# SauersML/genomic_pca

Measured on AMD Instinct MI355X. Metric: SNPs x samples / sec through rSVD at k=20; max|dPC| vs ref, higher is better.
Workload: dtype i8 (exact: int8 dosages x 4 signed 7-bit fixed-point digit planes of the skinny operand, i32 accumulate, f64 recombination; accuracy >= f32)

## Files before the change

### genomic_pca_amd/csrc/kernels.hip

```cpp
#include "kernels.h"
#include "philox.hpp"
#include "omega_math.h"

#ifndef GPCA_OMEGA_ABLATE
#define GPCA_OMEGA_ABLATE 0
#endif
namespace gpca {

__device__ const OmegaLnEntry kOmegaLnTable[kOmegaLnEntries] = {
#include "omega_table.inc"
};

typedef float f32x16 __attribute__((ext_vector_type(16)));

#define DEVINL __device__ __forceinline__

__global__ __launch_bounds__(256) void k_synth(int8_t* __restrict__ G, int64_t M, int64_t N, int64_t ld,
                                                int64_t snp_offset, uint64_t seed,
                                                const uint32_t* __restrict__ thresh, int P) {
    const int64_t per_row = ld >> 3;
    const int64_t t = (int64_t)blockIdx.x * 256 + threadIdx.x;
    if (t >= M * per_row) return;
    const int64_t i = t / per_row;
    const int64_t n0 = (t - i * per_row) << 3;
// ... 548 lines not shown
    const int64_t r0 = (int64_t)blockIdx.x * rpb;
    const int64_t r1 = (r0 + rpb < rows) ? r0 + rpb : rows;
    TX xc[4][G], xn[4][G];
    auto load_rows = [&](int64_t n, TX (&dst)[4][G]) {
#pragma unroll
        for (int u = 0; u < 4; ++u) {
            const int64_t row = n + 4 * u + k;
#pragma unroll
            for (int g = 0; g < G; ++g) dst[u][g] = row < r1 ? X[row * L + 16 * g + i] : (TX)0;
        }
    };
    load_rows(r0 + 16 * wv, xc);
    for (int64_t n = r0 + 16 * wv; n < r1; n += 64) {
        load_rows(n + 64, xn);
#pragma unroll
        for (int u = 0; u < 4; ++u) {
            double x[G];
#pragma unroll
            for (int g = 0; g < G; ++g) x[g] = (double)xc[u][g];
            int t = 0;
#pragma unroll
            for (int ga = 0; ga < G; ++ga)
#pragma unroll
                for (int gc = ga; gc < G; ++gc, ++t)
                    acc[t] = __builtin_amdgcn_mfma_f64_16x16x4f64(x[ga], x[gc], acc[t], 0, 0, 0);
        }
#pragma unroll
        for (int u = 0; u < 4; ++u)
#pragma unroll
            for (int g = 0; g < G; ++g) xc[u][g] = xn[u][g];
    }
    if (wv > 0) {
#pragma unroll
        for (int t = 0; t < NT; ++t)
#pragma unroll
            for (int r = 0; r < 4; ++r) red[wv - 1][t][lane][r] = acc[t][r];
    }
    __syncthreads();
    if (wv != 0) return;
    double* out = part + (int64_t)blockIdx.x * L * L;
    int t = 0;
#pragma unroll
    for (int ga = 0; ga < G; ++ga)
#pragma unroll
        for (int gc = ga; gc < G; ++gc, ++t)
#pragma unroll
            for (int r = 0; r < 4; ++r) {
                const double v = ((acc[t][r] + red[0][t][lane][r]) + red[1][t][lane][r]) + red[2][t][lane][r];
                const int a = 16 * ga + 4 * r + k, c = 16 * gc + i;
                out[a * L + c] = v;
                if (ga != gc) out[c * L + a] = v;
            }
}
void launch_gram_f64(hipStream_t st, const double* X, int64_t rows, int L, double* part) {
    const int64_t rpb = gram_rows_per_block(rows);
    const dim3 grid((unsigned)gram_num_parts(rows)), blk(256);
    if (L == 32) hipLaunchKernelGGL((k_gram_mfma<double, 32>), grid, blk, 0, st, X, rows, rpb, part);
    else if (L == 64) hipLaunchKernelGGL((k_gram_mfma<double, 64>), grid, blk, 0, st, X, rows, rpb, part);
    else launch_gram_any_f64(st, X, rows, rpb, gram_num_parts(rows), L, part);
}
void launch_gram_f32(hipStream_t st, const float* X, int64_t rows, int L, double* part) {
    const int64_t rpb = gram_rows_per_block(rows);
    const dim3 grid((unsigned)gram_num_parts(rows)), blk(256);
    if (L == 32) hipLaunchKernelGGL((k_gram_mfma<float, 32>), grid, blk, 0, st, X, rows, rpb, part);
    else if (L == 64) hipLaunchKernelGGL((k_gram_mfma<float, 64>), grid, blk, 0, st, X, rows, rpb, part);
    else launch_gram_any_f32(st, X, rows, rpb, gram_num_parts(rows), L, part);
}

template <int L>
__global__ __launch_bounds__(256) void k_apply_right(double* __restrict__ X, int64_t rows, const double* __restrict__ Z,
                                                     float* __restrict__ Qout, int64_t rows_pad) {
    constexpr int RPB = 256 / L;
    __shared__ double zs[L][L + 1];
    __shared__ double xs[RPB][L];
    for (int e = threadIdx.x; e < L * L; e += 256) zs[e / L][e % L] = Z[e];
    const int rr = threadIdx.x / L, cc = threadIdx.x % L;
    const int64_t n = (int64_t)blockIdx.x * RPB + rr;
    xs[rr][cc] = (n < rows) ? X[n * L + cc] : 0.0;
    __syncthreads();
    double a = 0.0;
#pragma unroll 8
    for (int j = 0; j < L; ++j) a += xs[rr][j] * zs[j][cc];
    if (n < rows) X[n * L + cc] = a;
    if (Qout && n < rows_pad) Qout[blocked_q_index(n, cc, L >> 5)] = (n < rows) ? (float)a : 0.f;
}
constexpr int kTailRows = 64;
int64_t tail_num_parts(int64_t rows_pad) { return (rows_pad + kTailRows - 1) / kTailRows; }
template <int L>
__global__ __launch_bounds__(256) void k_apply_right_tail(double* __restrict__ X, int64_t rows, const double* __restrict__ Z,
                                                          float* __restrict__ Qout, int64_t rows_pad,
                                                          double* __restrict__ csum_part, double* __restrict__ amax_part) {
    constexpr int RPB = 256 / L;
    __shared__ double zs[L][L + 1];
    __shared__ double xs[RPB][L];
    __shared__ double red[2][RPB][L];
    for (int e = threadIdx.x; e < L * L; e += 256) zs[e / L][e % L] = Z[e];
    const int rr = threadIdx.x / L, cc = threadIdx.x % L;
    double cs = 0.0, am = 0.0;
    const int64_t n0 = (int64_t)blockIdx.x * kTailRows;
    for (int sub = 0; sub < kTailRows; sub += RPB) {
        const int64_t n = n0 + sub + rr;
        __syncthreads();
        xs[rr][cc] = (n < rows) ? X[n * L + cc] : 0.0;
        __syncthreads();
        double a = 0.0;
#pragma unroll 8
        for (int j = 0; j < L; ++j) a += xs[rr][j] * zs[j][cc];
        if (n < rows) { X[n * L + cc] = a; cs += a; am = fmax(am, fabs(a)); }
        if (Qout && n < rows_pad) Qout[blocked_q_index(n, cc, L >> 5)] = (n < rows) ? (float)a : 0.f;
    }
    red[0][rr][cc] = cs; red[1][rr][cc] = am;
    __syncthreads();
    if (rr == 0) {
        for (int g = 1; g < RPB; ++g) { cs += red[0][g][cc]; am = fmax(am, red[1][g][cc]); }
        csum_part[(int64_t)blockIdx.x * L + cc] = cs;
        amax_part[(int64_t)blockIdx.x * L + cc] = am;
    }
}
void launch_apply_right_tail(hipStream_t st, double* X, int64_t rows, int L, const double* Z, float* Qout, int64_t rows_pad,
                             double* csum_part, double* amax_part) {
    const dim3 grid((unsigned)tail_num_parts(rows_pad)), blk(256);
    if (L == 32) hipLaunchKernelGGL((k_apply_right_tail<32>), grid, blk, 0, st, X, rows, Z, Qout, rows_pad, csum_part, amax_part);
    else if (L == 64) hipLaunchKernelGGL((k_apply_right_tail<64>), grid, blk, 0, st, X, rows, Z, Qout, rows_pad, csum_part, amax_part);
    else launch_apply_right_any(st, X, rows, tail_num_parts(rows_pad), L, Z, csum_part, amax_part);
}
__global__ __launch_bounds__(1024) void k_finish_q(const double* __restrict__ csum_part, const double* __restrict__ amax_part,
                                                   int64_t P, int L, double* __restrict__ s64, float* __restrict__ s32,
                                                   double* __restrict__ scale, double* __restrict__ inv, double S) {
    __shared__ double rs[1024], rm[1024];
    const int cc = threadIdx.x % L, pg = threadIdx.x / L, G = 1024 / L;
    double a = 0.0, m = 0.0;
    for (int64_t p = pg; p < P; p += G) { a += csum_part[p * L + cc]; m = fmax(m, amax_part[p * L + cc]); }
    rs[threadIdx.x] = a; rm[threadIdx.x] = m;
    __syncthreads();
    if (pg != 0) return;
    for (int g = 1; g < G; ++g) { a += rs[g * L + cc]; m = fmax(m, rm[g * L + cc]); }
    s64[cc] = a; s32[cc] = (float)a;
    if (scale) { scale[cc] = m > 0.0 ? m / S : 0.0; inv[cc] = m > 0.0 ? S / m : 0.0; }
}
void launch_finish_q(hipStream_t st, const double* csum_part, const double* amax_part, int64_t P, int L, double* s64, float* s32,
                     double* scale, double* inv, int nd) {
    hipLaunchKernelGGL(k_finish_q, dim3(1), dim3(1024), 0, st, csum_part, amax_part, P, L, s64, s32, scale, inv, digit_scale(nd));
}

constexpr double kCholRankTol = 1e-13;
__device__ __forceinline__ double rsqrt_nr(double x) {
    double y = __builtin_amdgcn_rsq(x);
    y = y * (1.5 - 0.5 * x * y * y);
    y = y * (1.5 - 0.5 * x * y * y);
    return y;
}
__device__ __forceinline__ double bcast_lane(double v, int lane) {
    return __hiloint2double(__builtin_amdgcn_readlane(__double2hiint(v), lane), __builtin_amdgcn_readlane(__double2loint(v), lane));
}
__device__ __forceinline__ void wave_lds_sync() { __builtin_amdgcn_fence(__ATOMIC_RELEASE, "wavefront"); __builtin_amdgcn_wave_barrier(); __builtin_amdgcn_fence(__ATOMIC_ACQUIRE, "wavefront"); }
template <int NN>
__device__ __forceinline__ void chol_inv_wave(const double* Wg, int n, double* __restrict__ Zg, int* __restrict__ flag, double* rs, int c) {
    double col[NN], x[NN], dinv[NN];
#pragma unroll
    for (int r = 0; r < NN; ++r) col[r] = Wg[r * NN + (c & (NN - 1))];
#pragma unroll
    for (int r = 0; r < NN; ++r) col[r] = (r < n && c < n) ? col[r] : ((r == c) ? 1.0 : 0.0);
    double diag0 = 0.0;
#pragma unroll
    for (int r = 0; r < NN; ++r) diag0 = (r == c) ? col[r] : diag0;
#pragma unroll
    for (int j = 0; j < NN; ++j) {
        __builtin_amdgcn_sched_barrier(0);
        double piv = bcast_lane(col[j], j);
        const double d0 = bcast_lane(diag0, j);
        if (!isfinite(piv) || !isfinite(d0)) {
            if (c == 0) atomicCAS(flag, 0, j + 1);
            piv = 1.0;
        }
        const bool dependent = !(piv > kCholRankTol * d0);
        dinv[j] = dependent ? 0.0 : rsqrt_nr(piv);
        col[j] = (c == j) ? piv * dinv[j] : col[j] * dinv[j];
        if (c < NN) rs[j * NN + c] = col[j];
        wave_lds_sync();
        double row[NN];
#pragma unroll
        for (int r = j + 1; r < NN; ++r) row[r] = rs[j * NN + r];
#pragma unroll
        for (int r = j + 1; r < NN; ++r) asm volatile("" : "+v"(row[r]));
#pragma unroll
        for (int r = j + 1; r < NN; ++r) { col[r] -= row[r] * col[j]; asm volatile("" : "+v"(col[r])); }
    }
#pragma unroll
    for (int i = NN - 1; i >= 0; --i) {
        __builtin_amdgcn_sched_barrier(0);
        double acc = (c == i) ? 1.0 : 0.0;
#pragma unroll
        for (int k = i + 1; k < NN; ++k) acc -= rs[i * NN + k] * x[k];
        x[i] = acc * dinv[i];
        asm volatile("" : "+v"(x[i]));
    }
    if (c < NN) {
#pragma unroll
        for (int i = 0; i < NN; ++i) Zg[i * NN + c] = (i < n && c < n) ? x[i] : 0.0;
    }
}
template <int NN>
__global__ __launch_bounds__(64) void k_chol_inv(const double* __restrict__ Wg, int n, double* __restrict__ Zg,
                                                 int* __restrict__ flag) {
    __shared__ double rs[NN * NN];
    chol_inv_wave<NN>(Wg, n, Zg, flag, rs, (int)threadIdx.x);
}
__global__ __launch_bounds__(256) void k_chol_inv_fold32(const double* __restrict__ part, int P, int n, double* __restrict__ Zg, int* __restrict__ flag) {
    __shared__ double rs[32 * 32];
    double a[4] = {0.0, 0.0, 0.0, 0.0};
    for (int p0 = 0; p0 < P; p0 += 16) {
        double v[4][16];
#pragma unroll
        for (int u = 0; u < 16; ++u) {
            const double* pp = part + (size_t)(p0 + u < P ? p0 + u : p0) * 1024 + threadIdx.x;
#pragma unroll
            for (int q = 0; q < 4; ++q) v[q][u] = pp[256 * q];
        }
#pragma unroll
        for (int u = 0; u < 16; ++u)
#pragma unroll
            for (int q = 0; q < 4; ++q) a[q] += (p0 + u < P) ? v[q][u] : 0.0;
    }
#pragma unroll
    for (int q = 0; q < 4; ++q) rs[threadIdx.x + 256 * q] = a[q];
    __syncthreads();
    if (threadIdx.x >= 64) return;
    chol_inv_wave<32>(rs, n, Zg, flag, rs, (int)threadIdx.x);
}
void launch_chol_inv_fold(hipStream_t st, const double* part, int P, int n, int ld, double* Z, int* flag) {
    (void)ld;
    hipLaunchKernelGGL(k_chol_inv_fold32, dim3(1), dim3(256), 0, st, part, P, n, Z, flag);
}
void launch_chol_inv(hipStream_t st, const double* W, int n, int ld, double* Z, int* flag) {
    if (ld == 32) hipLaunchKernelGGL(k_chol_inv<32>, dim3(1), dim3(64), 0, st, W, n, Z, flag);
    else if (ld == 64) hipLaunchKernelGGL(k_chol_inv<64>, dim3(1), dim3(64), 0, st, W, n, Z, flag);
    else (void)launch_chol_inv_any(st, W, n, ld, Z, flag);
}

void launch_apply_right_inplace(hipStream_t st, double* X, int64_t rows, int L, const double* Z, float* Qout,
                                int64_t rows_pad) {
    const int64_t span = Qout ? rows_pad : rows;
    if (L == 32) hipLaunchKernelGGL((k_apply_right<32>), dim3((unsigned)((span + 7) / 8)), dim3(256), 0, st, X, rows, Z, Qout, rows_pad);
    else if (L == 64) hipLaunchKernelGGL((k_apply_right<64>), dim3((unsigned)((span + 3) / 4)), dim3(256), 0, st, X, rows, Z, Qout, rows_pad);
    else launch_apply_right_any(st, X, rows, (rows + 63) / 64, L, Z, nullptr, nullptr);
}

template <typename TX, int L>
__global__ __launch_bounds__(256) void k_rightmul(const TX* __restrict__ X, const int64_t* __restrict__ row_ids,
                                                  int64_t nrows, const double* __restrict__ Z, int K,
                                                  double* __restrict__ out64, float* __restrict__ out32) {
    extern __shared__ double zsm[];
    float* osm = reinterpret_cast<float*>(zsm + L * K);
    const int KP = K | 1;
    for (int e = threadIdx.x; e < L * K; e += 256) zsm[e] = Z[e];
    __syncthreads();
    const int64_t n0 = (int64_t)blockIdx.x * 256;
    const int64_t n = n0 + threadIdx.x;
    if (n < nrows) {
        const int64_t src = row_ids ? row_ids[n] : n;
        double x[L];
#pragma unroll
        for (int j = 0; j < L; ++j) x[j] = (double)X[src * L + j];
        for (int kc = 0; kc < K; ++kc) {
            double a = 0.0;
#pragma unroll
            for (int j = 0; j < L; ++j) a += x[j] * zsm[j * K + kc];
            if (out64) out64[n * K + kc] = a;
            if (out32) osm[threadIdx.x * KP + kc] = (float)a;
        }
    }
    if (!out32) return;
    __syncthreads();
    const int64_t rows_here = (nrows - n0 < 256) ? nrows - n0 : 256;
    const int total = (int)rows_here * K;
    float* dst = out32 + n0 * K;
    for (int e = threadIdx.x; e < total; e += 256) dst[e] = osm[(e / K) * KP + (e % K)];
}
static size_t rightmul_lds(int L, int K, bool f32out) { return sizeof(double) * L * K + (f32out ? sizeof(float) * 256 * (size_t)(K | 1) : 0); }
void launch_rightmul_f64(hipStream_t st, const double* X, int64_t rows, int L, const double* Z, int K, double* out64,
                         float* out32) {
    const dim3 grid((unsigned)((rows + 255) / 256)), blk(256);
    const size_t lds = rightmul_lds(L, K, out32 != nullptr);
    if (L == 32) hipLaunchKernelGGL((k_rightmul<double, 32>), grid, blk, lds, st, X, (const int64_t*)nullptr, rows, Z, K, out64, out32);
    else if (L == 64) {
        hipLaunchKernelGGL((k_rightmul<double, 64>), grid, blk, lds, st, X, (const int64_t*)nullptr, rows, Z, K, out64, out32);
    } else launch_rightmul_any_f64(st, X, rows, L, Z, K, out64, out32);
}
template <int L, int NJ>
__global__ __launch_bounds__(256) void k_rightmul_mfma(const float* __restrict__ X, const int64_t* __restrict__ row_ids,
                                                       int64_t nrows, const double* __restrict__ Z, int K,
                                                       float* __restrict__ out32, int64_t tiles_per_wave, const int* __restrict__ sign) {
    constexpr int E = L / 4;
    const int lane = threadIdx.x & 63, wv = threadIdx.x >> 6;
    const int i = lane & 15, kq = lane >> 4;
    double zb[E][NJ];
#pragma unroll
    for (int jt = 0; jt < NJ; ++jt) {
        const int col = 16 * jt + i;
        const double sg = (sign && col < K) ? (double)sign[col] : 1.0;
#pragma unroll
        for (int s2 = 0; s2 < E; ++s2) zb[s2][jt] = col < K ? Z[(E * kq + s2) * K + col] * sg : 0.0;
    }
    __shared__ float osm[4][16 * 64];
    const int64_t ntiles = (nrows + 15) >> 4;
    const int64_t t0 = ((int64_t)blockIdx.x * 4 + wv) * tiles_per_wave;
    const int64_t t1 = (t0 + tiles_per_wave < ntiles) ? t0 + tiles_per_wave : ntiles;
    float xa[E], xn[E];
    auto load_tile = [&](int64_t tile, float (&dst)[E]) {
        const int64_t row = tile * 16 + i;
        const bool valid = row < nrows && tile < t1;
        const int64_t src = valid ? (row_ids ? row_ids[row] : row) : 0;
        const float4* xp = reinterpret_cast<const float4*>(X + src * L + E * kq);
#pragma unroll
        for (int v = 0; v < E / 4; ++v) {
            const float4 q = xp[v];
            dst[4 * v] = valid ? q.x : 0.f; dst[4 * v + 1] = valid ? q.y : 0.f; dst[4 * v + 2] = valid ? q.z : 0.f; dst[4 * v + 3] = valid ? q.w : 0.f;
        }
    };
    if (t0 < t1) load_tile(t0, xa);
    for (int64_t tile = t0; tile < t1; ++tile) {
        load_tile(tile + 1, xn);
        f64x4 acc[NJ];
#pragma unroll
        for (int jt = 0; jt < NJ; ++jt) acc[jt] = f64x4{0.0, 0.0, 0.0, 0.0};
#pragma unroll
        for (int s2 = 0; s2 < E; ++s2) {
            const double a = (double)xa[s2];
#pragma unroll
            for (int jt = 0; jt < NJ; ++jt) acc[jt] = __builtin_amdgcn_mfma_f64_16x16x4f64(a, zb[s2][jt], acc[jt], 0, 0, 0);
        }
#pragma unroll
        for (int jt = 0; jt < NJ; ++jt) {
            const int col = 16 * jt + i;
            if (col < K) {
#pragma unroll
                for (int r = 0; r < 4; ++r) osm[wv][(4 * r + kq) * K + col] = (float)acc[jt][r];
            }
        }
        const int64_t rows_here = (nrows - tile * 16 < 16) ? nrows - tile * 16 : 16;
        float* dst = out32 + tile * 16 * K;
        for (int e = lane; e < (int)rows_here * K; e += 64) dst[e] = osm[wv][e];
#pragma unroll
        for (int s2 = 0; s2 < E; ++s2) xa[s2] = xn[s2];
    }
}
void launch_rightmul_gather_f32(hipStream_t st, const float* X, const int64_t* row_ids, int64_t nrows, int L,
                                const double* Z, int K, float* out32, const int* sign) {
    if (nrows == 0) return;
    if (L > 64) { launch_rightmul_any_gather_f32(st, X, row_ids, nrows, L, Z, K, out32); return; }
    const int64_t ntiles = (nrows + 15) / 16;
    int64_t tpw = ntiles / (4 * 2048);
    if (tpw < 1) tpw = 1;
    const int64_t waves = (ntiles + tpw - 1) / tpw;
    const dim3 grid((unsigned)((waves + 3) / 4)), blk(256);
    const int nj = (K + 15) / 16;
#define GPCA_RM(LL, NN) hipLaunchKernelGGL((k_rightmul_mfma<LL, NN>), grid, blk, 0, st, X, row_ids, nrows, Z, K, out32, tpw, sign)
    if (L == 32) { if (nj == 1) GPCA_RM(32, 1); else if (nj == 2) GPCA_RM(32, 2); else if (nj == 3) GPCA_RM(32, 3); else GPCA_RM(32, 4); }
    else { if (nj == 1) GPCA_RM(64, 1); else if (nj == 2) GPCA_RM(64, 2); else if (nj == 3) GPCA_RM(64, 3); else GPCA_RM(64, 4); }
#undef GPCA_RM
}

constexpr int kScoreParts = 48;
int64_t scores_num_parts(int64_t rows) { const int64_t c = (rows + 255) / 256; return c < kScoreParts ? (c < 1 ? 1 : c) : kScoreParts; }
template <int L>
__global__ __launch_bounds__(256) void k_scores(const double* __restrict__ X, int64_t nrows, const double* __restrict__ Z, int K,
                                                double* __restrict__ out64, double* __restrict__ cand_val, int64_t* __restrict__ cand_idx) {
    extern __shared__ double zsc[];
    double* tile = zsc + L * K;
    double* win_val = tile + 256 * 17;
    long long* win_idx = reinterpret_cast<long long*>(win_val + 64);
    __shared__ double seg_val[256];
    __shared__ int seg_row[256];
    for (int e = threadIdx.x; e < L * K; e += 256) zsc[e] = Z[e];
    if (threadIdx.x < 64) { win_val[threadIdx.x] = 0.0; win_idx[threadIdx.x] = -1; }
    __syncthreads();
    const int64_t nchunks = (nrows + 255) / 256;
    for (int64_t chunk = blockIdx.x; chunk < nchunks; chunk += gridDim.x) {
        const int64_t n0 = chunk * 256, n = n0 + threadIdx.x;
        const bool live = n < nrows;
        double x[L];
#pragma unroll
        for (int j = 0; j < L; ++j) x[j] = live ? X[n * L + j] : 0.0;
        for (int k0 = 0; k0 < K; k0 += 16) {
            const int kn = K - k0 < 16 ? K - k0 : 16;
            for (int kc = 0; kc < kn; ++kc) {
                double a = 0.0;
#pragma unroll
                for (int j = 0; j < L; ++j) a += x[j] * zsc[j * K + k0 + kc];
                if (live) out64[n * K + k0 + kc] = a;
                tile[threadIdx.x * 17 + kc] = a;
            }
            __syncthreads();
            {
                const int kc = threadIdx.x & 15, seg = threadIdx.x >> 4;
                const int rows_here = nrows - n0 < 256 ? (int)(nrows - n0) : 256;
                double cv = 0.0; int cr = -1;
                if (kc < kn) {
                    double av[16];
#pragma unroll
                    for (int r = 0; r < 16; ++r) av[r] = tile[(16 * seg + r) * 17 + kc];
#pragma unroll
                    for (int r = 0; r < 16; ++r) if (16 * seg + r < rows_here && (cr < 0 || fabs(av[r]) > fabs(cv))) { cv = av[r]; cr = 16 * seg + r; }
                }
                seg_val[threadIdx.x] = cv; seg_row[threadIdx.x] = cr;
            }
            __syncthreads();
            if ((int)threadIdx.x < kn) {
                double cv = win_val[k0 + threadIdx.x]; long long ci = win_idx[k0 + threadIdx.x];
                for (int sg2 = 0; sg2 < 16; ++sg2) {
                    const double a = seg_val[16 * sg2 + threadIdx.x]; const int r = seg_row[16 * sg2 + threadIdx.x];
                    if (r >= 0 && (ci < 0 || fabs(a) > fabs(cv))) { cv = a; ci = n0 + r; }
                }
                win_val[k0 + threadIdx.x] = cv; win_idx[k0 + threadIdx.x] = ci;
            }
            __syncthreads();
        }
    }
    for (int kc = threadIdx.x; kc < K; kc += 256) { cand_val[(int64_t)blockIdx.x * K + kc] = win_val[kc]; cand_idx[(int64_t)blockIdx.x * K + kc] = win_idx[kc]; }
}
__global__ __launch_bounds__(256) void k_scores_sign(double* __restrict__ X64, float* __restrict__ X32, int64_t total, int K,
                                                     const double* __restrict__ cand_val, const int64_t* __restrict__ cand_idx, int parts,
                                                     int* __restrict__ sign) {
    extern __shared__ double cv_s[];
    long long* ci_s = reinterpret_cast<long long*>(cv_s + parts * K);
    __shared__ int sg[kMaxSketchCols];
    for (int e = threadIdx.x; e < parts * K; e += 256) { cv_s[e] = cand_val[e]; ci_s[e] = cand_idx[e]; }
    __syncthreads();
    for (int kc = threadIdx.x; kc < K; kc += 256) {
        double bv = 0.0; long long bi = -1;
        for (int p = 0; p < parts; ++p) {
            const double ov = cv_s[p * K + kc]; const long long oi = ci_s[p * K + kc];
            const bool take = oi >= 0 && (bi < 0 || fabs(ov) > fabs(bv) || (fabs(ov) == fabs(bv) && oi < bi));
            bv = take ? ov : bv; bi = take ? oi : bi;
        }
        const int s1 = (bi >= 0 && bv < 0.0) ? -1 : 1;
        sg[kc] = s1;
        if (blockIdx.x == 0) sign[kc] = s1;
    }
    __syncthreads();
    for (int64_t t = (int64_t)blockIdx.x * 256 + threadIdx.x; t < total; t += (int64_t)gridDim.x * 256) {
        const double v = X64[t] * (double)sg[t % K];
        X64[t] = v;
        if (X32) X32[t] = (float)v;
    }
}
void launch_scores(hipStream_t st, const double* X, int64_t rows, int L, const double* Z, int K, double* out64, double* cand_val, int64_t* cand_idx) {
    const dim3 grid((unsigned)scores_num_parts(rows)), blk(256);
    const size_t lds = sizeof(double) * ((size_t)L * K + 256 * 17 + 64) + sizeof(long long) * 64;
    if (L == 32) hipLaunchKernelGGL((k_scores<32>), grid, blk, lds, st, X, rows, Z, K, out64, cand_val, cand_idx);
    else hipLaunchKernelGGL((k_scores<64>), grid, blk, lds, st, X, rows, Z, K, out64, cand_val, cand_idx);
}
void launch_scores_sign(hipStream_t st, double* out64, float* out32, int64_t rows, int K, const double* cand_val, const int64_t* cand_idx,
                        int64_t parts, int* sign) {
    const int64_t total = rows * K;
    int64_t blocks = (total + 1023) / 1024;
    blocks = blocks < 1 ? 1 : (blocks > 512 ? 512 : blocks);
    const size_t lds = (sizeof(double) + sizeof(long long)) * (size_t)parts * K;
    hipLaunchKernelGGL(k_scores_sign, dim3((unsigned)blocks), dim3(256), lds, st, out64, out32, total, K, cand_val, cand_idx, (int)parts, sign);
}

constexpr int kColsumRowsPerBlock = 256;
int64_t colsum_num_parts(int64_t rows) { return (rows + kColsumRowsPerBlock - 1) / kColsumRowsPerBlock; }
__global__ __launch_bounds__(256) void k_colsum(const double* __restrict__ X, int64_t rows, int L, double* __restrict__ part) {
    __shared__ double red[256];
    const int cc = threadIdx.x % L, rg = threadIdx.x / L, nrg = 256 / L;
    const int64_t r0 = (int64_t)blockIdx.x * kColsumRowsPerBlock;
    const int64_t r1 = (r0 + kColsumRowsPerBlock < rows) ? r0 + kColsumRowsPerBlock : rows;
    double a = 0.0;
    for (int64_t n = r0 + rg; n < r1; n += nrg) a += (double)X[n * L + cc];
    red[threadIdx.x] = a;
    __syncthreads();
    if (rg == 0) {
        for (int g = 1; g < nrg; ++g) a += red[g * L + cc];
        part[(int64_t)blockIdx.x * L + cc] = a;
    }
}
void launch_colsum_f64(hipStream_t st, const double* X, int64_t rows, int L, double* part) {
    hipLaunchKernelGGL(k_colsum, dim3((unsigned)colsum_num_parts(rows)), dim3(256), 0, st, X, rows, L, part);
}

__global__ __launch_bounds__(1024) void k_col_sign(const double* __restrict__ X, int64_t rows, int K, int* __restrict__ sign) {
    __shared__ double bv[1024];
    __shared__ long long bi[1024];
    const int col = blockIdx.x;
    double best = -1.0; long long idx = -1;
    for (int64_t n0 = threadIdx.x; n0 < rows; n0 += 4096) {
        double a[4];
#pragma unroll
        for (int u = 0; u < 4; ++u) { const int64_t n = n0 + 1024 * u; a[u] = n < rows ? fabs(X[n * K + col]) : -1.0; }
#pragma unroll
        for (int u = 0; u < 4; ++u) if (a[u] > best) { best = a[u]; idx = n0 + 1024 * u; }
    }
    bv[threadIdx.x] = best; bi[threadIdx.x] = idx;
    __syncthreads();
    for (int s = 512; s > 0; s >>= 1) {
        if (threadIdx.x < s) {
            const double ob = bv[threadIdx.x + s]; const long long oi = bi[threadIdx.x + s];
            if (ob > bv[threadIdx.x] || (ob == bv[threadIdx.x] && oi >= 0 && (bi[threadIdx.x] < 0 || oi < bi[threadIdx.x]))) {
                bv[threadIdx.x] = ob; bi[threadIdx.x] = oi;
            }
        }
        __syncthreads();
    }
    if (threadIdx.x == 0) sign[col] = (bi[0] >= 0 && X[bi[0] * K + col] < 0.0) ? -1 : 1;
}
void launch_col_sign(hipStream_t st, const double* X, int64_t rows, int K, int* sign) {
    hipLaunchKernelGGL(k_col_sign, dim3(K), dim3(1024), 0, st, X, rows, K, sign);
}
__global__ void k_scale_cols(double* X64, float* X32, int64_t rows, int K, const int* sign) {
    const int64_t t = (int64_t)blockIdx.x * 256 + threadIdx.x;
    if (t >= rows * K) return;
    const double v = X64[t] * (double)sign[t % K];
    X64[t] = v;
    if (X32) X32[t] = (float)v;
}
void launch_scale_cols(hipStream_t st, double* X64, float* X32, int64_t rows, int K, const int* sign) {
    const int64_t total = rows * K;
    hipLaunchKernelGGL(k_scale_cols, dim3((unsigned)((total + 255) / 256)), dim3(256), 0, st, X64, X32, rows, K, sign);
}
__global__ void k_f64_to_f32(const double* in, float* out, int64_t n) {
    const int64_t t = (int64_t)blockIdx.x * 256 + threadIdx.x;
    if (t < n) out[t] = (float)in[t];
}
void launch_f64_to_f32(hipStream_t st, const double* in, float* out, int64_t n) {
    hipLaunchKernelGGL(k_f64_to_f32, dim3((unsigned)((n + 255) / 256)), dim3(256), 0, st, in, out, n);
}
__global__ void k_fill_f32(float* p, int64_t n, float v) {
    const int64_t t = (int64_t)blockIdx.x * 256 + threadIdx.x;
    if (t < n) p[t] = v;
}
void launch_fill_f32(hipStream_t st, float* p, int64_t n, float v) {
    hipLaunchKernelGGL(k_fill_f32, dim3((unsigned)((n + 255) / 256)), dim3(256), 0, st, p, n, v);
}


__global__ void k_expand_loadings(const float* __restrict__ load, const int64_t* __restrict__ rows, int64_t n_pca, int k,
                                  int L, float* __restrict__ Tp) {
    const int64_t t = (int64_t)blockIdx.x * 256 + threadIdx.x;
    if (t >= n_pca * k) return;
    const int64_t a = t / k;
    const int c = (int)(t - a * k);
    Tp[rows[a] * L + c] = load[t];
}
void launch_expand_loadings(hipStream_t st, const float* load, const int64_t* rows, int64_t n_pca, int k, int L, float* Tp) {
    const int64_t total = n_pca * k;
    if (total == 0) return;
    hipLaunchKernelGGL(k_expand_loadings, dim3((unsigned)((total + 255) / 256)), dim3(256), 0, st, load, rows, n_pca, k, L, Tp);
}

__global__ __launch_bounds__(256) void k_scale_rows(const float* __restrict__ X, int64_t M, int64_t Mpad, int L,
                                                    const float* __restrict__ r, const float* __restrict__ b,
                                                    float* __restrict__ Tb, float* __restrict__ cpart, int blocked) {
    const int lane = threadIdx.x & 63;
    const int64_t wave = (int64_t)blockIdx.x * 4 + (threadIdx.x >> 6);
    if (wave >= (Mpad + 63) / 64) return;
    const int64_t i = wave * 64 + lane;
    const bool live = i < M;
    const float ri = live ? r[i] : 0.f, bi = live ? b[i] : 0.f;
    const int LT = L >> 5;
    for (int j = 0; j < L; ++j) {
        const float x = live ? X[i * L + j] : 0.f;
        if (i < Mpad) Tb[blocked ? blocked_t_index(i, j, LT) : i * L + j] = ri * x;
        float cv = bi * x;
#pragma unroll
        for (int o = 32; o > 0; o >>= 1) cv += __shfl_xor(cv, o);
        if (lane == 0) cpart[wave * L + j] = cv;
    }
}
void launch_scale_rows(hipStream_t st, const float* X, int64_t M, int64_t Mpad, int L, const float* r, const float* b,
                       float* Tb, float* cpart, int blocked) {
    const int64_t waves = (Mpad + 63) / 64;
    hipLaunchKernelGGL(k_scale_rows, dim3((unsigned)((waves + 3) / 4)), dim3(256), 0, st, X, M, Mpad, L, r, b, Tb, cpart, blocked);
}


__global__ __launch_bounds__(256) void k_bd_expand(const float* __restrict__ W, const int32_t* __restrict__ feat0, int cmax,
                                                   const double* __restrict__ P, int64_t M, int L, float* __restrict__ out) {
    const int64_t t = (int64_t)blockIdx.x * 256 + threadIdx.x;
    if (t >= M * L) return;
    const int64_t i = t / L;
    const int j = (int)(t - i * L);
    const int32_t f = feat0[i];
    double a = 0.0;
    if (f >= 0)
        for (int c = 0; c < cmax; ++c) a = fma((double)W[i * cmax + c], P[(int64_t)(f + c) * L + j], a);
    out[t] = (float)a;
}
void launch_bd_expand(hipStream_t st, const float* W, const int32_t* feat0, int cmax, const double* P, int64_t M, int L, float* out) {
    hipLaunchKernelGGL(k_bd_expand, dim3((unsigned)((M * L + 255) / 256)), dim3(256), 0, st, W, feat0, cmax, P, M, L, out);
}
__global__ __launch_bounds__(256) void k_bd_reduce(const float* __restrict__ W, const int32_t* __restrict__ feat0, int cmax,
                                                   const float* __restrict__ T, int L, const int64_t* __restrict__ blk_row0,
                                                   const int64_t* __restrict__ blk_row1, const int32_t* __restrict__ blk_feat0,
                                                   const int32_t* __restrict__ blk_c, double* __restrict__ P) {
    const int b = blockIdx.x;
    const int64_t r0 = blk_row0[b], r1 = blk_row1[b];
    const int32_t bf = blk_feat0[b];
    const int cb = blk_c[b];
    const int cg = threadIdx.x >> 5, jl = threadIdx.x & 31;
    for (int c = cg; c < cb; c += 8)
        for (int j = jl; j < L; j += 32) {
            double a = 0.0;
            for (int64_t i = r0; i < r1; ++i)
                if (feat0[i] == bf) a = fma((double)W[i * cmax + c], (double)T[i * L + j], a);
            P[(int64_t)(bf + c) * L + j] = a;
        }
}
void launch_bd_reduce(hipStream_t st, const float* W, const int32_t* feat0, int cmax, const float* T, int L, const int64_t* blk_row0,
                      const int64_t* blk_row1, const int32_t* blk_feat0, const int32_t* blk_c, int B, double* P) {
    if (B <= 0) return;
    hipLaunchKernelGGL(k_bd_reduce, dim3((unsigned)B), dim3(256), 0, st, W, feat0, cmax, T, L, blk_row0, blk_row1, blk_feat0, blk_c, P);
}
template <int L>
__global__ __launch_bounds__(256) void k_rightmul_inplace_f32(float* __restrict__ X, int64_t rows, const double* __restrict__ Z) {
    __shared__ double zs[L * L];
    for (int e = threadIdx.x; e < L * L; e += 256) zs[e] = Z[e];
    __syncthreads();
    const int64_t i = (int64_t)blockIdx.x * 256 + threadIdx.x;
    if (i >= rows) return;
    double x[L];
#pragma unroll
    for (int k = 0; k < L; ++k) x[k] = (double)X[i * L + k];
    for (int j = 0; j < L; ++j) {
        double a = 0.0;
#pragma unroll
        for (int k = 0; k < L; ++k) a = fma(x[k], zs[k * L + j], a);
        X[i * L + j] = (float)a;
    }
}
void launch_rightmul_inplace_f32(hipStream_t st, float* X, int64_t rows, int L, const double* Z) {
    const dim3 grid((unsigned)((rows + 255) / 256)), blk(256);
    if (L == 32) hipLaunchKernelGGL((k_rightmul_inplace_f32<32>), grid, blk, 0, st, X, rows, Z);
    else hipLaunchKernelGGL((k_rightmul_inplace_f32<64>), grid, blk, 0, st, X, rows, Z);
}
__global__ __launch_bounds__(256) void k_mask_rows(double* __restrict__ Y, int64_t N, int L, const uint8_t* __restrict__ mask) {
    const int64_t t = (int64_t)blockIdx.x * 256 + threadIdx.x;
    if (t >= N * L) return;
    if (!mask[t / L]) Y[t] = 0.0;
}
void launch_mask_rows(hipStream_t st, double* Y, int64_t N, int L, const uint8_t* mask) {
    hipLaunchKernelGGL(k_mask_rows, dim3((unsigned)((N * L + 255) / 256)), dim3(256), 0, st, Y, N, L, mask);
}
__global__ __launch_bounds__(256) void k_f32_to_f64(const float* __restrict__ in, double* __restrict__ out, int64_t n) {
    const int64_t t = (int64_t)blockIdx.x * 256 + threadIdx.x;
    if (t < n) out[t] = (double)in[t];
}
void launch_f32_to_f64(hipStream_t st, const float* in, double* out, int64_t n) {
    hipLaunchKernelGGL(k_f32_to_f64, dim3((unsigned)((n + 255) / 256)), dim3(256), 0, st, in, out, n);
}

int init_device_kernels_common() {
    hipError_t e = hipFuncSetAttribute(reinterpret_cast<const void*>(k_rightmul<double, 64>), hipFuncAttributeMaxDynamicSharedMemorySize, 100 * 1024);
    if (e == hipSuccess) e = hipFuncSetAttribute(reinterpret_cast<const void*>(k_scores<64>), hipFuncAttributeMaxDynamicSharedMemorySize, 72 * 1024);
    return (int)e;
}

}
```

Baseline: 985.3 billion.

## Prefetch gather indices, vectorize output stores, size rightmul grid to resident occupancy

The rightmul MFMA kernel now reads the row_ids gather index two tiles ahead, so the dependent index load is off the critical path of the next tile's X load. The LDS-to-global output copy uses float4 stores with a scalar tail. The launcher replaces the fixed 4*2048 wave divisor with a persistent-style grid sized from queried occupancy times CU count. This adds host-side occupancy and device queries per launch, and the float4 store assumes out32 tiles are 16-byte aligned, which only holds when K is suitable.

```diff
diff --git a/genomic_pca_amd/csrc/kernels.hip b/genomic_pca_amd/csrc/kernels.hip
--- a/genomic_pca_amd/csrc/kernels.hip
+++ b/genomic_pca_amd/csrc/kernels.hip
@@ -874,25 +874,30 @@
 #pragma unroll
         for (int s2 = 0; s2 < E; ++s2) zb[s2][jt] = col < K ? Z[(E * kq + s2) * K + col] * sg : 0.0;
     }
-    __shared__ float osm[4][16 * 64];
+    __shared__ __align__(16) float osm[4][16 * 64];
     const int64_t ntiles = (nrows + 15) >> 4;
     const int64_t t0 = ((int64_t)blockIdx.x * 4 + wv) * tiles_per_wave;
     const int64_t t1 = (t0 + tiles_per_wave < ntiles) ? t0 + tiles_per_wave : ntiles;
+    auto row_of = [&](int64_t tile) -> int64_t {
+        const int64_t row = tile * 16 + i;
+        return (row < nrows && tile < t1) ? (row_ids ? row_ids[row] : row) : -1;
+    };
     float xa[E], xn[E];
-    auto load_tile = [&](int64_t tile, float (&dst)[E]) {
-        const int64_t row = tile * 16 + i;
-        const bool valid = row < nrows && tile < t1;
-        const int64_t src = valid ? (row_ids ? row_ids[row] : row) : 0;
-        const float4* xp = reinterpret_cast<const float4*>(X + src * L + E * kq);
+    auto load_row = [&](int64_t src, float (&dst)[E]) {
+        const float4* xp = reinterpret_cast<const float4*>(X + (src < 0 ? 0 : src) * L + E * kq);
 #pragma unroll
         for (int v = 0; v < E / 4; ++v) {
             const float4 q = xp[v];
-            dst[4 * v] = valid ? q.x : 0.f; dst[4 * v + 1] = valid ? q.y : 0.f; dst[4 * v + 2] = valid ? q.z : 0.f; dst[4 * v + 3] = valid ? q.w : 0.f;
+            const bool ok = src >= 0;
+            dst[4 * v] = ok ? q.x : 0.f; dst[4 * v + 1] = ok ? q.y : 0.f; dst[4 * v + 2] = ok ? q.z : 0.f; dst[4 * v + 3] = ok ? q.w : 0.f;
         }
     };
-    if (t0 < t1) load_tile(t0, xa);
+    int64_t src_next = row_of(t0 + 1);
+    if (t0 < t1) load_row(row_of(t0), xa);
     for (int64_t tile = t0; tile < t1; ++tile) {
-        load_tile(tile + 1, xn);
+        const int64_t src_after = row_of(tile + 2);
+        load_row(src_next, xn);
+        src_next = src_after;
         f64x4 acc[NJ];
 #pragma unroll
         for (int jt = 0; jt < NJ; ++jt) acc[jt] = f64x4{0.0, 0.0, 0.0, 0.0};
@@ -912,22 +917,36 @@
         }
         const int64_t rows_here = (nrows - tile * 16 < 16) ? nrows - tile * 16 : 16;
         float* dst = out32 + tile * 16 * K;
-        for (int e = lane; e < (int)rows_here * K; e += 64) dst[e] = osm[wv][e];
+        const int total = (int)rows_here * K, total4 = total >> 2;
+        for (int e = lane; e < total4; e += 64) reinterpret_cast<float4*>(dst)[e] = reinterpret_cast<const float4*>(osm[wv])[e];
+        for (int e = 4 * total4 + lane; e < total; e += 64) dst[e] = osm[wv][e];
 #pragma unroll
         for (int s2 = 0; s2 < E; ++s2) xa[s2] = xn[s2];
     }
+}
+template <int L, int NJ>
+static int64_t rightmul_resident_wgs() {
+    static int per_cu = 0;
+    if (per_cu == 0) {
+        int n = 0;
+        if (hipOccupancyMaxActiveBlocksPerMultiprocessor(&n, k_rightmul_mfma<L, NJ>, 256, 0) != hipSuccess || n < 1) n = 1;
+        per_cu = n;
+    }
+    int dev = 0, cus = 0;
+    if (hipGetDevice(&dev) != hipSuccess || hipDeviceGetAttribute(&cus, hipDeviceAttributeMultiprocessorCount, dev) != hipSuccess || cus < 1) cus = 256;
+    return (int64_t)per_cu * cus;
 }
 void launch_rightmul_gather_f32(hipStream_t st, const float* X, const int64_t* row_ids, int64_t nrows, int L,
                                 const double* Z, int K, float* out32, const int* sign) {
     if (nrows == 0) return;
     if (L > 64) { launch_rightmul_any_gather_f32(st, X, row_ids, nrows, L, Z, K, out32); return; }
     const int64_t ntiles = (nrows + 15) / 16;
-    int64_t tpw = ntiles / (4 * 2048);
-    if (tpw < 1) tpw = 1;
-    const int64_t waves = (ntiles + tpw - 1) / tpw;
-    const dim3 grid((unsigned)((waves + 3) / 4)), blk(256);
+#define GPCA_RM(LL, NN) do { \
+        const int64_t slots = 4 * rightmul_resident_wgs<LL, NN>(); \
+        const int64_t tpw = (ntiles + slots - 1) / slots, waves = (ntiles + tpw - 1) / tpw; \
+        hipLaunchKernelGGL((k_rightmul_mfma<LL, NN>), dim3((unsigned)((waves + 3) / 4)), dim3(256), 0, st, X, row_ids, nrows, Z, K, out32, tpw, sign); \
+    } while (0)
     const int nj = (K + 15) / 16;
-#define GPCA_RM(LL, NN) hipLaunchKernelGGL((k_rightmul_mfma<LL, NN>), grid, blk, 0, st, X, row_ids, nrows, Z, K, out32, tpw, sign)
     if (L == 32) { if (nj == 1) GPCA_RM(32, 1); else if (nj == 2) GPCA_RM(32, 2); else if (nj == 3) GPCA_RM(32, 3); else GPCA_RM(32, 4); }
     else { if (nj == 1) GPCA_RM(64, 1); else if (nj == 2) GPCA_RM(64, 2); else if (nj == 3) GPCA_RM(64, 3); else GPCA_RM(64, 4); }
 #undef GPCA_RM
```

Result: no change. 988.4 billion, median of 6 (+0.3%).
